# flyakon/DeepPhysiNet

Hardware: AMD Instinct MI355X
Metric: collocation-points/sec (fwd+PDE-Jacobian+bwd) (higher is better)
Workload: dtype bf16x2 (hi+lo split bf16 MFMA operands), fp32 accumulate

## Files before the change

### deepphysinet_amd/csrc/dpn_fwd_tiles.h

```cpp
#pragma once

namespace ts {
constexpr int kVecFloats = kNumVecs * 256 + 4;
template <int NS>
struct Cfg {
    static constexpr int kXBytes = 16 * 2 * NS * 1024;
    static constexpr int kVecOff = kXBytes;
    static constexpr int kRedOff = kVecOff + kVecFloats * 4;
    static constexpr int kLdsBytes = kRedOff + 4 * 64 * 4;
};

DEV void barrier_lds() {
    __builtin_amdgcn_fence(__ATOMIC_RELEASE, "workgroup", "local");
    __builtin_amdgcn_s_barrier();
    __builtin_amdgcn_fence(__ATOMIC_ACQUIRE, "workgroup", "local");
}

struct NoSide { DEV void operator()(int) const {} };

#ifdef TS_ABL_NOSINCOS
template <int NS> DEV void ts_sincos(float th, float& s, float& c) { s = th; c = th * 0.5f; }
#else
template <int NS> DEV void ts_sincos(float th, float& s, float& c) { sincos_t<NS>(th, s, c); }
#endif
// ... 181 lines not shown
#pragma unroll
    for (int q = 0; q < 4; ++q) {
        float s, co;
        ts_sincos<NS>(xi * a.freqs[8 * (ks & 3) + 4 * h + q], s, co);
        frag_set2<NS>(f, q, s, co);
    }
}
template <int NS, class Args>
DEV void pe6_frag(Frag<NS>& f, const Args& a, const int ks, const int h, const int64_t pc, const float g = 1.0f) {
    const float v = a.coord_data[pc * 6 + (ks >> 1)];
#pragma unroll
    for (int q = 0; q < 4; ++q) {
        float s, co;
        ts_sincos<NS>(v * a.freqs[32 + 8 * (ks & 1) + 4 * h + q], s, co);
        frag_set2<NS>(f, q, g * s, g * co);
    }
}
template <int NS, class Args>
DEV void pe6_frag_dot(Frag<NS>& f, const Args& a, const int ks, const int h, const int64_t pc, const float* bv, float& dot) {
    const float v = a.coord_data[pc * 6 + (ks >> 1)];
    const f32x4* b4 = reinterpret_cast<const f32x4*>(bv + 16 * ks + 8 * h);
    const f32x4 b0 = b4[0], b1 = b4[1];
    const float bb[8] = {b0[0], b0[1], b0[2], b0[3], b1[0], b1[1], b1[2], b1[3]};
#pragma unroll
    for (int q = 0; q < 4; ++q) {
        float s, co;
        ts_sincos<NS>(v * a.freqs[32 + 8 * (ks & 1) + 4 * h + q], s, co);
        frag_set2<NS>(f, q, s, co);
        dot = fmaf(s, bb[2 * q], dot);
        dot = fmaf(co, bb[2 * q + 1], dot);
    }
}
template <int NS, class Args>
DEV void z0_frag(Frag<NS>& f, const Args& a, const int ks, const int h, const int64_t pc, const float g, const float gjc) {
    const int c = ks >> 2;
    const float* src = (c == 0) ? a.x : (c == 1) ? a.y : a.t;
    const float d1 = (c == 0) ? a.geo.dx : (c == 1) ? a.geo.dy : a.geo.pred_t_span;
    const float d2 = (c == 0) ? a.geo.lon_m1 : (c == 1) ? a.geo.lat_m1 : 1.0f;
    const float xi = src[pc] / d1 / d2;
#pragma unroll
    for (int q = 0; q < 4; ++q) {
        const float fr = a.freqs[8 * (ks & 3) + 4 * h + q];
        float s, co;
        ts_sincos<NS>(xi * fr, s, co);
        const float gf = gjc * fr;
        frag_set2<NS>(f, q, fmaf(g, s, gf * co), fmaf(g, co, -gf * s));
    }
}
template <int NS, class Args>
DEV void dpe_tile(float (&d)[16], const Args& a, const int c, const int t, const int h, const int64_t pc) {
    const float* src = (c == 0) ? a.x : (c == 1) ? a.y : a.t;
    const float d1 = (c == 0) ? a.geo.dx : (c == 1) ? a.geo.dy : a.geo.pred_t_span;
    const float d2 = (c == 0) ? a.geo.lon_m1 : (c == 1) ? a.geo.lat_m1 : 1.0f;
    const float xi = src[pc] / d1 / d2;
#pragma unroll
    for (int rp = 0; rp < 8; ++rp) {
        const int r = 2 * rp;
        const float fr = a.freqs[8 * ((2 * t + (r >> 3)) & 3) + 4 * h + ((r & 7) >> 1)];
        float s, co;
        ts_sincos<NS>(xi * fr, s, co);
        d[r] = fr * co;
        d[r + 1] = -fr * s;
    }
}
template <int NS, class Args>
DEV void z0_frag_derivs(Frag<NS>& f, const Args& a, const int ks, const int h, const int64_t pc, const float g, const float gjc, const float ghc) {
    const int c = ks >> 2;
    const float* src = (c == 0) ? a.x : (c == 1) ? a.y : a.t;
    const float d1 = (c == 0) ? a.geo.dx : (c == 1) ? a.geo.dy : a.geo.pred_t_span;
    const float d2 = (c == 0) ? a.geo.lon_m1 : (c == 1) ? a.geo.lat_m1 : 1.0f;
    const float xi = src[pc] / d1 / d2;
#pragma unroll
    for (int q = 0; q < 4; ++q) {
        const float fr = a.freqs[8 * (ks & 3) + 4 * h + q];
        float s, co;
        ts_sincos<NS>(xi * fr, s, co);
        const float gf = gjc * fr;
        const float gs = fmaf(-ghc * fr, fr, g);
        frag_set2<NS>(f, q, fmaf(gs, s, gf * co), fmaf(gs, co, -gf * s));
// ... 38 lines not shown
```

### deepphysinet_amd/csrc/dpn_layout.h

```cpp
#pragma once

#if defined(__HIPCC__)
#define DPN_HD __host__ __device__ constexpr
#else
#define DPN_HD constexpr
#endif

namespace dpn {

constexpr int kNets = 6;
constexpr int kHidden = 256;
constexpr int kPe = 192;
constexpr int kW1Stride = 193;
constexpr int kW2Stride = 257;

DPN_HD int drow32(int r, int h) { return (r & 3) + 8 * (r >> 2) + 4 * h; }
DPN_HD int chain_ch(int ks, int h, int e) { return 16 * ks + 8 * (e >> 2) + 4 * h + (e & 3); }

DPN_HD int pe3_angle(int ks, int h, int e) { return 8 * ks + 4 * h + (e >> 1); }
DPN_HD int pe3_ch(int ks, int h, int e) { return (pe3_angle(ks, h, e) & 31) * 6 + (e & 1) * 3 + (pe3_angle(ks, h, e) >> 5); }
DPN_HD int pe6_ch(int ks, int h, int e) { return (pe3_angle(ks, h, e) & 15) * 12 + (e & 1) * 6 + (pe3_angle(ks, h, e) >> 4); }

DPN_HD int gpe_row_to_pe3_ch(int rho) {
    const int T = rho >> 5, i = rho & 31;
    const int r = (i & 3) + 4 * (i >> 3), h = (i >> 2) & 1;
    return pe3_ch(2 * T + (r >> 3), h, r & 7);
}

constexpr int kS0 = 0;
constexpr int kS1 = kS0 + 8 * 12;
constexpr int kS2 = kS1 + 8 * 28;
constexpr int kS3 = kS2 + 8 * 16;
constexpr int kS4 = kS3 + 8 * 16;
constexpr int kS5 = kS4 + 8 * 16;
constexpr int kPackKB = kS5 + 6 * 16;
enum { kVecB1 = 0, kVecCvec, kVecBf1, kVecU, kVecWo, kVecB2BdE_unused, kNumVecs = 6 };
DPN_HD long pack_bytes_per_net(int ns) { return (long)kPackKB * 1024 * ns + kNumVecs * 1024 + 16; }

constexpr int kF0 = kS0, kFA = kS1, kFB = kS1 + 8 * 16, kFAT = kS2, kF5 = kS5;
static_assert(kFB + 8 * 12 == kS2 && kFAT + 8 * 16 == kS3, "fused form fits the block");
enum { kVecC2 = kVecCvec, kVecA2 = kVecBf1, kVecBv = kVecB2BdE_unused };

DPN_HD bool wgrad_coop_is_y(int ns, int wave, int j) { return j < ns || (j < 2 * ns && wave < 4); }
DPN_HD int wgrad_coop_piece(int ns, int issue, int wave, int j) {
    const int xlo = issue - 2 * ns, xhi = (16 - 4 * xlo) / 4;
    if (j < ns) return 16 + 12 * j + wave;
    if (wave < 4) return j < 2 * ns ? 16 + 12 * (j - ns) + 8 + wave : xlo * wave + (j - 2 * ns);
    return j - ns < xhi ? 4 * xlo + xhi * (wave - 4) + (j - ns) : -1;
}

}
```

### deepphysinet_amd/csrc/dpn_point.hip

```cpp
#include "dpn_point_common.h"

template <int NS>
struct Frag {
    u32x4 w[NS];
};
template <int NS>
DEV void frag_set2(Frag<NS>& f, const int p, float a, float b) {
    const u32 hi = pack2(a, b);
    f.w[0][p] = hi;
    if constexpr (NS == 2) f.w[1][p] = pack2(a - bf_lo(hi), b - bf_hi(hi));
}


DEV void sincos_precise(float th, float& s, float& c) {
    const float k = rintf(th * 0.63661977236758134f);
    float r = fmaf(k, -1.5707963705062866f, th);
    r = fmaf(k, 4.371138828673793e-08f, r);
    const float r2 = r * r;
    float sp = fmaf(r2, 2.7183114939898219064e-6f, -1.9839334836096632576e-4f);
    sp = fmaf(sp, r2, 8.3333293858894631756e-3f);
    sp = fmaf(sp, r2, -1.6666666641626524100e-1f);
    sp = fmaf(sp * r2, r, r);
    float cp = fmaf(r2, 2.4433157826443582e-5f, -1.3887316255057415e-3f);
    cp = fmaf(cp, r2, 4.1666645683529456e-2f);
// ... 273 lines not shown
    }
}
DEV float lds_read_f32(unsigned addr) {
    float r;
    asm volatile("ds_read_b32 %0, %1\n\ts_waitcnt lgkmcnt(0)" : "=&v"(r) : "v"(addr) : "memory");
    return r;
}

DEV void store_d_as_k(const KMat& m, int net, int ns, int s, int64_t tile32, int ct, int lane, const f32x16& d) {
    uint4 a, b;
    a.x = pack2(d[0], d[1]); a.y = pack2(d[2], d[3]); a.z = pack2(d[4], d[5]); a.w = pack2(d[6], d[7]);
    b.x = pack2(d[8], d[9]); b.y = pack2(d[10], d[11]); b.z = pack2(d[12], d[13]); b.w = pack2(d[14], d[15]);
    typedef __attribute__((ext_vector_type(4))) unsigned int u32x4_t;
#ifdef TS_ABL_NOSTORE
    asm volatile("" ::"v"(a.x), "v"(a.y), "v"(a.z), "v"(a.w), "v"(b.x), "v"(b.y), "v"(b.z), "v"(b.w));
    return;
#endif
    __builtin_nontemporal_store(u32x4_t{a.x, a.y, a.z, a.w}, reinterpret_cast<u32x4_t*>(kmat_ptr(m, net, ns, s, tile32, ct, lane, 0)));
    __builtin_nontemporal_store(u32x4_t{b.x, b.y, b.z, b.w}, reinterpret_cast<u32x4_t*>(kmat_ptr(m, net, ns, s, tile32, ct, lane, 1)));
}
template <int NS, int NSTORE>
DEV void store_tile_k(const KMat& m, int net, int64_t tile32, int ct, const Lane& L, const Frag<NS>& f0, const Frag<NS>& f1, bool partial) {
#pragma unroll
    for (int s = 0; s < NSTORE; ++s) {
        u32x4 a0 = f0.w[s], a1 = f1.w[s];
        if (partial && !L.valid) { a0 = (u32x4)0u; a1 = (u32x4)0u; }
        f32x16 d = (f32x16)0.f;
        d = mfma(as_bf(a0), as_bf(L.idA), d);
        d = mfma(as_bf(a1), as_bf(L.idB), d);
        store_d_as_k(m, net, NSTORE, s, tile32, ct, L.lane, d);
    }
}

struct FwdArgs {
    const float *x, *y, *t, *coord_data, *freqs, *pe_in;
    int64_t n, n_pad;
    DpnGeometry geo;
    const char* packed;
    float* out_n;
    float* jac_n;
    void* saved;
    const float* ref;
#ifdef DPN_TIMELINE
    unsigned* timeline;
#endif
};

#ifdef DPN_TIMELINE
#define DPN_STAMP(I)                                                                                          \
    do {                                                                                                      \
        unsigned long long t_;                                                                                \
        asm volatile("s_memtime %0\n\ts_waitcnt lgkmcnt(0)" : "=s"(t_)::"memory");                            \
        asm volatile("v_writelane_b32 %0, %1, %2" : "+v"(tl) : "s"((u32)t_), "n"(I));                         \
    } while (0)
#else
#define DPN_STAMP(I) do { } while (0)
#endif

#ifdef DPN_FWD_PHASES
#define DPN_PH_AFTER_MMA do { u32 c4_; DPN_PH_CLOCK(c4_); pipe.ph[3] += c4_ - pipe.pc0; pipe.pc0 = c4_; } while (0)
#else
#define DPN_PH_AFTER_MMA do { } while (0)
#endif
#define DPN_STEP(C, NK, SWAP, ACT, ACC, EPI_PREV)                                    \
    do {                                                                             \
        DPN_STAMP(2 + (C));                                                          \
// ... 161 lines not shown
```

### deepphysinet_amd/csrc/dpn_point_common.h

```cpp
#pragma once
#include "dpn_device.h"

DEV void dma16(const char* gsrc_lane, char* lds_wave_base) {
    __builtin_amdgcn_global_load_lds((const __attribute__((address_space(1))) void*)(gsrc_lane),
                                     (__attribute__((address_space(3))) void*)(lds_wave_base), 16, 0, 0);
}
template <int OFF> DEV void dma16_at(const char* gsrc_lane, char* lds_wave_base) {
    __builtin_amdgcn_global_load_lds((const __attribute__((address_space(1))) void*)(gsrc_lane),
                                     (__attribute__((address_space(3))) void*)(lds_wave_base), 16, OFF, 0);
}
DEV void dma16_nt(const char* gsrc_lane, char* lds_wave_base) {
    __builtin_amdgcn_global_load_lds((const __attribute__((address_space(1))) void*)(gsrc_lane),
                                     (__attribute__((address_space(3))) void*)(lds_wave_base), 16, 0, 2);
}
DEV void dma4(const char* gsrc_lane, char* lds_wave_base) {
    __builtin_amdgcn_global_load_lds((const __attribute__((address_space(1))) void*)(gsrc_lane),
                                     (__attribute__((address_space(3))) void*)(lds_wave_base), 4, 0, 0);
}
template <int N> DEV void wait_vmcnt() { asm volatile("s_waitcnt vmcnt(%0)" ::"n"(N) : "memory"); }

struct KMat {
    char* base;
    int64_t tiles32;
    int ct_per_tile;
};
DEV char* kmat_ptr(const KMat& m, int net, int ns, int s, int64_t tile32, int ct, int lane, int kk) {
    return m.base + (((int64_t)net * ns + s) * m.tiles32 + tile32) * (m.ct_per_tile * 2048) + ((kk * m.ct_per_tile + ct) * 64 + lane) * 16;
}

struct SavedView {
    KMat T1;
    KMat M2;
    uint4* m1;
};
DEV SavedView saved_view(void* base, int64_t n_pad, int ns) {
    SavedView s;
    char* b = reinterpret_cast<char*>(base);
    const int64_t mat = (int64_t)kNets * ns * n_pad * 512;
    const int64_t tiles32 = n_pad / 32;
    s.T1 = KMat{b, tiles32, 8};
    s.M2 = KMat{b + mat, tiles32, 8};
    s.m1 = reinterpret_cast<uint4*>(b + mat + (int64_t)kNets * n_pad * 512);
    return s;
}
DPN_HD int64_t saved_state_bytes(int64_t n_pad, int ns) { return (int64_t)kNets * ns * n_pad * 512 + (int64_t)kNets * n_pad * 512 + (int64_t)kNets * n_pad * 32; }

struct OperandView {
    KMat Z1;
    KMat Z0;
    KMat PE6;
    float* gnet;
};
DEV OperandView operand_view(void* base, int64_t n_pad, int ns) {
    OperandView o;
    char* b = reinterpret_cast<char*>(base);
    const int64_t m256 = (int64_t)kNets * ns * n_pad * 512, m192 = (int64_t)kNets * ns * n_pad * 384, t192 = (int64_t)ns * n_pad * 384;
    const int64_t tiles32 = n_pad / 32;
    o.Z1 = KMat{b, tiles32, 8};
    o.Z0 = KMat{b + m256, tiles32, 6};
    o.PE6 = KMat{b + m256 + m192, tiles32, 6};
    o.gnet = reinterpret_cast<float*>(b + m256 + m192 + t192);
    return o;
}
static inline int64_t operand_bytes(int64_t n_pad, int ns) { return (int64_t)kNets * ns * n_pad * 512 + (int64_t)(kNets + 1) * ns * n_pad * 384 + (int64_t)kNets * n_pad * 4 + 1024; }

static inline int64_t pad_points(int64_t n) { return ((n + 127) / 128) * 128; }
static inline bool use_tiles(const char* knob, int prec, bool has_pe_in) {
    const char* force = getenv(knob);
    return (force ? (force[0] == 't') : (prec == 2)) && !has_pe_in;
}
```

### deepphysinet_amd/csrc/dpn_ring_kernels.inc

```

template <int NS>
#if DPN_DERIV
__global__ __launch_bounds__(256, 1) void dpn_fwd_deriv_kernel(FwdArgs a, float* hess_n, float* d3_n) {
#else
__global__ __launch_bounds__(256, 1) void dpn_fwd_kernel(FwdArgs a) {
#endif
    __shared__ __attribute__((aligned(16))) char lds_w[Pipe<NS>::kRing * Pipe<NS>::kSlotBytes];

    const int net = blockIdx.y;
    const int wave = threadIdx.x >> 6;
    const int64_t tile32 = (int64_t)blockIdx.x * 4 + wave;
    const char* pk = a.packed + (long)net * pack_bytes_per_net(NS);
    __shared__ __attribute__((aligned(16))) float lds_vec_store[kNumVecs * 256 + 4];
#ifdef DPN_TIMELINE
    u32 tl = 0;
    DPN_STAMP(0);
#endif
    {
        const float* gv = reinterpret_cast<const float*>(pk + (long)kPackKB * 1024 * NS);
        for (int i = threadIdx.x; i < kNumVecs * 256 + 4; i += 256) lds_vec_store[i] = gv[i];
    }
    const unsigned lds_vec = (unsigned)(uintptr_t)(__attribute__((address_space(3))) float*)lds_vec_store;
    Lane L;
    lane_init(L, a.x, a.y, a.t, a.n, a.freqs, a.geo, tile32);
// ... 227 lines not shown
    __shared__ __attribute__((aligned(16))) float lds_vec_store[kNumVecs * 256 + 4];
    {
        const float* gv = reinterpret_cast<const float*>(pk + (long)kPackKB * 1024 * NS);
        for (int i = threadIdx.x; i < kNumVecs * 256 + 4; i += 256) lds_vec_store[i] = gv[i];
    }
    const unsigned lds_vec = (unsigned)(uintptr_t)(__attribute__((address_space(3))) float*)lds_vec_store;
    Lane L;
    lane_init(L, a.x, a.y, a.t, a.n, a.freqs, a.geo, tile32);
    const int h = L.h;
    const int64_t pc = L.valid ? L.pt : (a.n - 1);
    float cd6[6];
#pragma unroll
    for (int c = 0; c < 6; ++c) cd6[c] = a.coord_data[pc * 6 + c];
    const float gsc = a.g_scale ? a.g_scale[0] : 1.0f;
    const float g = L.valid ? gsc * a.g_out[pc * 6 + net] : 0.f;
    float gj[3] = {0.f, 0.f, 0.f};
    if (a.g_jxi && L.valid) {
#pragma unroll
        for (int c = 0; c < 3; ++c) gj[c] = gsc * a.g_jxi[(pc * 6 + net) * 3 + c];
    }
#if DPN_DERIV
    float gh[3] = {0.f, 0.f, 0.f};
    if (g_hxi && L.valid) {
#pragma unroll
        for (int c = 0; c < 3; ++c) gh[c] = gsc * g_hxi[(pc * 6 + net) * 3 + c];
    }
#endif
    SavedView sv = saved_view(a.saved, a.n_pad, NS);
    OperandView ov = operand_view(a.operands, a.n_pad, NS);
    const int64_t tiles32 = a.n_pad / 32;
    const uint4 m1v = sv.m1[((int64_t)net * tiles32 + tile32) * 64 + L.lane];
    const u32 m1w[4] = {m1v.x, m1v.y, m1v.z, m1v.w};
    if (h == 0) ov.gnet[(int64_t)net * a.n_pad + tile32 * 32 + L.j] = g;

    Pipe<NS> pipe;
    __syncthreads();
    pipe.init(pk, lds_w, 8);
    pipe.prime();

    f32x16 acc[8];
    Frag<NS> actA[16];
#ifdef DPN_TIMELINE
    u32 tl = 0;
#endif
    auto epi1 = [&](const int T) __attribute__((always_inline)) {
#pragma unroll
        for (int r = 0; r < 16; r += 2) {
            const u32 bits = m1w[T >> 1] >> (16 * (T & 1) + r);
            frag_set2<NS>(actA[2 * T + (r >> 3)], (r & 7) >> 1, (bits & 1u) ? acc[T][r] : 0.f, (bits & 2u) ? acc[T][r + 1] : 0.f);
        }
        store_tile_k<NS, NS>(ov.Z1, net, tile32, T, L, actA[2 * T], actA[2 * T + 1], false);
    };
    {
        Frag<NS> z0[12];
        if (net == 0) {
            build_pe6<NS>(L, cd6, z0, 1.0f);
#pragma unroll
            for (int ct = 0; ct < 6; ++ct) store_tile_k<NS, NS>(ov.PE6, 0, tile32, ct, L, z0[2 * ct], z0[2 * ct + 1], false);
        }
        if (a.pe_in) load_pe3<NS>(a.pe_in + pc * kPe, h, z0, g);
#if DPN_DERIV
        else build_z0_derivs<NS>(L, z0, g, gj, gh);
#else
        else build_pe3<NS, true>(L, z0, g, gj);
#endif
#pragma unroll
        for (int ct = 0; ct < 6; ++ct) store_tile_k<NS, NS>(ov.Z0, net, tile32, ct, L, z0[2 * ct], z0[2 * ct + 1], false);
#pragma unroll
        for (int T = 0; T < 8; ++T) {
            acc_init_vec(acc[T], lds_vec, kVecB1, h, T, g);
            if (T == 0) DPN_STEP(T, 12, false, z0, acc[T], (void)0);
            else DPN_STEP(T, 12, false, z0, acc[T], epi1(T - 1));
        }
        epi1(7);
        pipe.drain();
    }
}
```

### deepphysinet_amd/csrc/dpn_tiles_kernels.inc

```

template <int NS>
#if DPN_DERIV
__global__ __launch_bounds__(256, 2) void dpn_fwd_tiles_deriv_kernel(FwdArgs a, float* hess_n, float* d3_n) {
#else
__global__ __launch_bounds__(256, 2) void dpn_fwd_tiles_kernel(FwdArgs a) {
#endif
    using C = ts::Cfg<NS>;
    __shared__ __attribute__((aligned(16))) char lds[C::kLdsBytes];
    const int net = blockIdx.y;
    const int w = __builtin_amdgcn_readfirstlane(threadIdx.x >> 6);
    const int lane = threadIdx.x & 63, j = lane & 31, h = lane >> 5;
    const char* pk = a.packed + (long)net * pack_bytes_per_net(NS);
#if TS_PRIO == 2
    __builtin_amdgcn_s_setprio(1);
#endif
    TS_STAMP(0);
    float* vec = reinterpret_cast<float*>(lds + C::kVecOff);
    float* red = reinterpret_cast<float*>(lds + C::kRedOff);
    char* xl = lds + lane * 16;
    {
        const u32x4* gv = reinterpret_cast<const u32x4*>(pk + (long)kPackKB * 1024 * NS);
        static_assert(ts::kVecFloats % 4 == 0 && ts::kVecFloats / 4 <= 512, "vector block");
        const int i0 = threadIdx.x, i1 = threadIdx.x + 256;
        const u32x4 v0 = gv[i0];
// ... 289 lines not shown
    const int lane = threadIdx.x & 63, j = lane & 31, h = lane >> 5;
    TS_STAMP(0);
    const char* pk = a.packed + (long)net * pack_bytes_per_net(NS);
#if TS_PRIO == 2
    __builtin_amdgcn_s_setprio(1);
#endif
    float* vec = reinterpret_cast<float*>(lds + kXBytes) - kVecB1 * 256;
    char* xl = lds + lane * 16;
    {
        const float* gv = reinterpret_cast<const float*>(pk + (long)kPackKB * 1024 * NS) + kVecB1 * 256;
        reinterpret_cast<float*>(lds + kXBytes)[threadIdx.x] = gv[threadIdx.x];
    }
    auto chunk = [&](const int kb) __attribute__((always_inline)) { return pk + (long)kb * 1024 * NS; };
    ts::Head<NS, 2> H;
    ts::gemm_head<NS, 12, 2>(chunk(kS0 + 2 * w * 12), lane, H);
    const int64_t tile0 = (int64_t)blockIdx.x * 2;
    const int64_t tiles32 = a.n_pad / 32;
    int64_t pc[2];
    float g[2];
    const float gsc = a.g_scale ? a.g_scale[0] : 1.0f;
#pragma unroll
    for (int p = 0; p < 2; ++p) {
        const int64_t pt = (tile0 + p) * 32 + j;
        const bool valid = pt < a.n;
        pc[p] = valid ? pt : (a.n - 1);
        g[p] = valid ? gsc * a.g_out[pc[p] * 6 + net] : 0.f;
    }
    const ts::Ident I = ts::make_ident(j, h);
    SavedView sv = saved_view(a.saved, a.n_pad, NS);
    OperandView ov = operand_view(a.operands, a.n_pad, NS);
    u32 m1w[2];
#pragma unroll
    for (int p = 0; p < 2; ++p) m1w[p] = reinterpret_cast<const u32*>(sv.m1 + ((int64_t)net * tiles32 + tile0 + p) * 64 + lane)[w];
    if (w == 0) {
        const int64_t pt = (tile0 + h) * 32 + j;
        ov.gnet[(int64_t)net * a.n_pad + pt] = (pt < a.n) ? gsc * a.g_out[pt * 6 + net] : 0.f;
    }
#pragma unroll
    for (int uu = 0; uu < 3; ++uu) {
        const int u = 3 * w + uu, ct = u >> 1, p = u & 1;
        const float gp = p ? g[1] : g[0];
        const int64_t pcp = p ? pc[1] : pc[0];
        float gjc = 0.f;
        if (a.g_jxi && ((tile0 + p) * 32 + j) < a.n) gjc = gsc * a.g_jxi[(pcp * 6 + net) * 3 + (ct >> 1)];
        Frag<NS> f0, f1;
#if DPN_DERIV
        float ghc = 0.f;
        if (g_hxi && ((tile0 + p) * 32 + j) < a.n) ghc = gsc * g_hxi[(pcp * 6 + net) * 3 + (ct >> 1)];
        ts::z0_frag_derivs<NS>(f0, a, 2 * ct, h, pcp, gp, gjc, ghc);
        ts::z0_frag_derivs<NS>(f1, a, 2 * ct + 1, h, pcp, gp, gjc, ghc);
#else
        ts::z0_frag<NS>(f0, a, 2 * ct, h, pcp, gp, gjc);
        ts::z0_frag<NS>(f1, a, 2 * ct + 1, h, pcp, gp, gjc);
#endif
        ts::x_store<NS>(xl, 2 * ct, p, f0);
        ts::x_store<NS>(xl, 2 * ct + 1, p, f1);
        ts::save_tile_k<NS, NS>(ov.Z0, net, tile0 + p, ct, lane, I, false, f0, f1);
    }
    TS_STAMP(1);
    ts::barrier_lds();
    TS_STAMP(2);
    f32x16 acc[2][2];
#pragma unroll
    for (int t = 0; t < 2; ++t)
#pragma unroll
        for (int p = 0; p < 2; ++p) ts::acc_init(acc[t][p], vec, kVecB1, h, 2 * w + t, g[p]);
    ts::gemm<NS, 12, 2, false, ts::NoSide, false>(chunk(kS0 + 2 * w * 12), xl, lane, H, acc);
    TS_STAMP(3);
#pragma unroll
    for (int t = 0; t < 2; ++t)
#pragma unroll
        for (int p = 0; p < 2; ++p) {
            Frag<NS> F0, F1;
#pragma unroll
            for (int r = 0; r < 16; r += 2) {
                const u32 bits = m1w[p] >> (16 * t + r);
                frag_set2<NS>(r < 8 ? F0 : F1, (r & 7) >> 1, (bits & 1u) ? acc[t][p][r] : 0.f, (bits & 2u) ? acc[t][p][r + 1] : 0.f);
            }
            ts::save_tile_k<NS, NS>(ov.Z1, net, tile0 + p, 2 * w + t, lane, I, false, F0, F1);
        }
    TS_STAMP(4);
    if (net != 0) return;
#pragma unroll
    for (int uu = 0; uu < 3; ++uu) {
        const int u = 3 * w + uu, ct = u >> 1, p = u & 1;
        const int64_t pcp = p ? pc[1] : pc[0];
        Frag<NS> f0, f1;
        ts::pe6_frag<NS>(f0, a, 2 * ct, h, pcp);
        ts::pe6_frag<NS>(f1, a, 2 * ct + 1, h, pcp);
// ... 5 lines not shown
```

### deepphysinet_amd/csrc/dpn_wgrad.hip

```cpp
#include <type_traits>

#include "dpn_point_common.h"

DEV u16 f2bf(float x) {
    unsigned u = __float_as_uint(x);
    u += 0x7FFFu + ((u >> 16) & 1u);
    return (u16)(u >> 16);
}
DEV float bf2f(u16 b) { return __uint_as_float(((unsigned)b) << 16); }

struct PackArgs {
    DpnNetPtrs net[kNets];
    char* packed;
    int ns;
    int form;
    int n_fields;
    long heads_stride, evec_stride, packed_stride;
};
DEV DpnNetPtrs pack_net(const PackArgs& a, const int net, const int field) {
    DpnNetPtrs P = a.net[net];
    P.w1b1 += field * a.heads_stride;
    P.w2b2 += field * a.heads_stride;
    P.evec += field * a.evec_stride;
    return P;
// ... 224 lines not shown
#ifdef DPN_WGRAD_PHASES
    unsigned* phases;
#endif
};
#ifdef DPN_WGRAD_PHASES
#define DPN_WG_CLOCK(V) do { unsigned long long t_; asm volatile("s_memtime %0\n\ts_waitcnt lgkmcnt(0)" : "=s"(t_)::"memory"); V = (u32)t_; } while (0)
#else
#define DPN_WG_CLOCK(V) do { } while (0)
#endif

template <int NS, int PROD>
struct WgradShape {
    static constexpr int nct = PROD < 2 ? 8 : 6;
    static constexpr int nsx = PROD == 3 ? NS : 1;
    static constexpr int kX = nsx * 16384, kYPlane = nct * 2048, kY = NS * kYPlane;
    static constexpr int kPieces = (kX + kY) / 1024;
    static constexpr int kIssue = (kPieces + 7) / 8;
    static constexpr int kPad = kIssue * 8 - kPieces;
    static constexpr int kGOff = kX + kY;
    static constexpr int kPadOff = kGOff + 8 * 256;
    static constexpr int kSlot = kPadOff + (kPad ? 1024 : 0);
    static constexpr int PER_TILE = kIssue + 1;
    static constexpr int RING = (160 * 1024) / kSlot < 5 ? (160 * 1024) / kSlot : 5;
};
template <int NS>
constexpr int wgrad_lds_bytes() {
    int m = 0;
    const int v[3] = {WgradShape<NS, 1>::RING * WgradShape<NS, 1>::kSlot, WgradShape<NS, 2>::RING * WgradShape<NS, 2>::kSlot,
                      WgradShape<NS, 3>::RING * WgradShape<NS, 3>::kSlot};
    for (int k = 0; k < 3; ++k) m = v[k] > m ? v[k] : m;
    return m;
}

template <int NS, int PROD>
DEV void wgrad_body(const WgradArgs& a, char* lds, const int split, const int net) {
    using S = WgradShape<NS, PROD>;
    constexpr int nct = S::nct, nsx = S::nsx, kSlot = S::kSlot, RING = S::RING, PER_TILE = S::PER_TILE, ncol = nct * 32;
    const int64_t tiles = a.n_pad / 32;
    const int64_t per = (tiles + a.splits[PROD] - 1) / a.splits[PROD];
    const int64_t t0 = (int64_t)split * per;
    int64_t t1 = t0 + per < tiles ? t0 + per : tiles;
    if (t1 < t0) t1 = t0;

    const int lane = threadIdx.x & 63, wave = __builtin_amdgcn_readfirstlane(threadIdx.x >> 6);
#ifdef DPN_WGRAD_2X4_ONLY
    constexpr bool kWide = true;
#else
    constexpr bool kWide = nct == 8;
#endif
    constexpr int MT = kWide ? 4 : 2, NT = kWide ? 2 : 3;
    const int wm = kWide ? wave >> 2 : wave >> 1, wn = kWide ? wave & 3 : wave & 1;
    const int i = lane & 31, h = lane >> 5;
    const bool active = wn * NT < nct;
    SavedView sv = saved_view(a.saved, a.n_pad, NS);
    OperandView ov = operand_view(a.operands, a.n_pad, NS);
    const char* xb = (PROD == 3) ? sv.T1.base : sv.M2.base;
    static_assert(PROD >= 1 && PROD <= 3, "products: 1 = M2^T Z1, 2 = M2^T G6, 3 = T1^T Z0");
    const char* yb = (PROD == 1) ? ov.Z1.base : (PROD == 2) ? ov.PE6.base : ov.Z0.base;
    const int64_t ynet = (PROD == 2) ? 0 : net;
    const float* gnet = ov.gnet + (int64_t)net * a.n_pad;

    constexpr bool kCoop = PROD == 2;
    static_assert(!kCoop || (2 * nct == 12 && nsx == 1 && S::kIssue >= 2 * NS), "product 2: 12 column pairs over 8 waves");
    const bool two_pairs = wave < 4;
    const char* pbase[S::kIssue];
    int pstride[S::kIssue], pdst[S::kIssue];
#pragma unroll
    for (int j = 0; j < S::kIssue; ++j) {
        int q = wave + 8 * j;
        if constexpr (kCoop) q = wgrad_coop_piece(NS, S::kIssue, wave, j);
        if (S::kPad && (kCoop ? q < 0 : q >= S::kPieces)) {
            pbase[j] = xb + ((int64_t)net * nsx * tiles + (t0 < tiles ? t0 : 0)) * 16384; pstride[j] = 0; pdst[j] = S::kPadOff;
        } else if (q < nsx * 16) {
            pbase[j] = xb + ((int64_t)net * nsx + q / 16) * tiles * 16384 + (q % 16) * 1024; pstride[j] = 16384; pdst[j] = q * 1024;
        } else {
            const int qy = q - nsx * 16;
            pbase[j] = yb + (ynet * NS + qy / (2 * nct)) * tiles * S::kYPlane + (qy % (2 * nct)) * 1024; pstride[j] = S::kYPlane; pdst[j] = q * 1024;
        }
    }
    auto issue = [&](int64_t tile, int slot) __attribute__((always_inline)) {
        char* sl = lds + slot * kSlot;
#pragma unroll
        for (int j = 0; j < S::kIssue; ++j) {
            if (kCoop && wgrad_coop_is_y(NS, wave, j)) dma16(pbase[j] + tile * pstride[j] + lane * 16, sl + pdst[j]);
            else dma16_nt(pbase[j] + tile * pstride[j] + lane * 16, sl + pdst[j]);
        }
        dma4(reinterpret_cast<const char*>(gnet + tile * 32) + lane * 4, sl + S::kGOff + wave * 256);
    };

    f32x16 acc[MT][NT];
#pragma unroll
    for (int m = 0; m < MT; ++m)
#pragma unroll
        for (int n2 = 0; n2 < NT; ++n2) acc[m][n2] = (f32x16)0.f;
    float vecA[MT], vecB[NT], gsum = 0.f;
#pragma unroll
    for (int m = 0; m < MT; ++m) vecA[m] = 0.f;
#pragma unroll
    for (int n2 = 0; n2 < NT; ++n2) vecB[n2] = 0.f;
    auto owns_row = [&](const int m) __attribute__((always_inline)) { return (kWide && nct == 6) ? wn == m % 3 : wn == m; };
    auto owns_col = [&](const int n2) __attribute__((always_inline)) { return wm == n2; };

    const unsigned lds_base = (unsigned)(uintptr_t)(__attribute__((address_space(3))) char*)lds;
    auto rd128 = [&](u32x4& v, const unsigned addr) __attribute__((always_inline)) {
        asm volatile("ds_read_b128 %0, %1" : "=v"(v) : "v"(addr) : "memory");
    };
    auto compute = [&](const int slot_) __attribute__((always_inline)) {
        const unsigned buf = lds_base + slot_ * kSlot;
        const unsigned gl = buf + S::kGOff + wave * 256;
        constexpr int KB = (NS == 1) ? 2 : 1;
        u32x4 gqa[KB][2], faa[KB][nsx][MT], fba[KB][NS][NT];
        const unsigned baseG = gl + h * 16;
        const unsigned baseA = buf + wm * (MT * 1024) + lane * 16, baseB = buf + S::kX + wn * (NT * 1024) + lane * 16;
        auto rd128o = [&](u32x4& v, const unsigned base, const int off) __attribute__((always_inline)) {
            asm volatile("ds_read_b128 %0, %1 offset:%2" : "=v"(v) : "v"(base), "i"(off) : "memory");
        };
        auto issue_reads = [&](const int kk, const int b) __attribute__((always_inline)) {
            if constexpr (!kCoop) {
                rd128o(gqa[b][0], baseG, 64 * kk);
                rd128o(gqa[b][1], baseG, 64 * kk + 32);
            }
#pragma unroll
            for (int s2 = 0; s2 < nsx; ++s2)
#pragma unroll
                for (int m = 0; m < MT; ++m) rd128o(faa[b][s2][m], baseA, s2 * 16384 + (kk * 8 + m) * 1024);
#pragma unroll
            for (int s2 = 0; s2 < NS; ++s2)
#pragma unroll
                for (int n2 = 0; n2 < NT; ++n2) rd128o(fba[b][s2][n2], baseB, s2 * S::kYPlane + (kk * nct + n2) * 1024);
        };
        constexpr int kReads = (kCoop ? 0 : 2) + MT * nsx + NT * NS;
        if constexpr (NS == 1) { issue_reads(0, 0); issue_reads(1, 1); }
#pragma unroll
        for (int kk = 0; kk < 2; ++kk) {
            const int b = (NS == 1) ? kk : 0;
            if constexpr (NS == 2) issue_reads(kk, 0);
            u32x4 (&fa)[nsx][MT] = faa[b];
            u32x4 (&fb)[NS][NT] = fba[b];
            u32x4& gq0 = gqa[b][0];
            u32x4& gq1 = gqa[b][1];
            if (NS == 1 && kk == 0) asm volatile("s_waitcnt lgkmcnt(%0)" :: "n"(kReads) : "memory");
            else asm volatile("s_waitcnt lgkmcnt(0)" ::: "memory");
            if constexpr (kCoop) gq0 = gq1 = (u32x4)0u;
            else asm volatile("" : "+v"(gq0), "+v"(gq1));
            asm volatile("" : "+v"(fa[0][0]), "+v"(fa[0][1]), "+v"(fb[0][0]), "+v"(fb[0][1]));
            if constexpr (MT == 4) asm volatile("" : "+v"(fa[0][2]), "+v"(fa[0][3]));
            if constexpr (NT == 3) asm volatile("" : "+v"(fb[0][2]));
            if constexpr (NS == 2) asm volatile("" : "+v"(fb[1][0]), "+v"(fb[1][1]));
            if constexpr (NS == 2 && NT == 3) asm volatile("" : "+v"(fb[1][2]));
            if constexpr (nsx == 2) asm volatile("" : "+v"(fa[1][0]), "+v"(fa[1][1]));
            if constexpr (nsx == 2 && MT == 4) asm volatile("" : "+v"(fa[1][2]), "+v"(fa[1][3]));
            const float gp[8] = {__uint_as_float(gq0[0]), __uint_as_float(gq0[1]), __uint_as_float(gq0[2]), __uint_as_float(gq0[3]),
                                 __uint_as_float(gq1[0]), __uint_as_float(gq1[1]), __uint_as_float(gq1[2]), __uint_as_float(gq1[3])};
            if (PROD == 1 && wave == 0 && i == 0) {
#pragma unroll
                for (int e = 0; e < 8; ++e) gsum += gp[e];
            }
#pragma unroll
            for (int m = 0; m < MT; ++m) {
                if (owns_row(m) && PROD != 2) {
                    float d = 0.f;
#pragma unroll
                    for (int s2 = 0; s2 < nsx; ++s2) {
#pragma unroll
                        for (int p = 0; p < 4; ++p) { d = fmaf(bf_lo(fa[s2][m][p]), gp[2 * p], d); d = fmaf(bf_hi(fa[s2][m][p]), gp[2 * p + 1], d); }
                    }
                    vecA[m] += d;
                }
#pragma unroll
                for (int n2 = 0; n2 < NT; ++n2) {
                    if constexpr (NS == 2) {
                        acc[m][n2] = mfma(as_bf(fa[0][m]), as_bf(fb[1][n2]), acc[m][n2]);
                        if constexpr (nsx == 2) acc[m][n2] = mfma(as_bf(fa[1][m]), as_bf(fb[0][n2]), acc[m][n2]);
                    }
                    acc[m][n2] = mfma(as_bf(fa[0][m]), as_bf(fb[0][n2]), acc[m][n2]);
                }
// ... 16 lines not shown
    auto form = [&](const int slot_) __attribute__((always_inline)) {
        const unsigned buf = lds_base + slot_ * kSlot;
        const unsigned baseG = buf + S::kGOff + wave * 256 + h * 16, baseY = buf + S::kX + wave * 1024 + lane * 16;
        auto pair = [&](auto q_) __attribute__((always_inline)) {
            constexpr int q = decltype(q_)::value;
            const unsigned ay = baseY + q * 8192, ag = baseG + ((wave + 8 * q) >= nct ? 64 : 0);
            u32x4 t[2], gq0, gq1;
            rd128(gq0, ag);
            asm volatile("ds_read_b128 %0, %1 offset:32" : "=v"(gq1) : "v"(ag) : "memory");
            rd128(t[0], ay);
            if constexpr (NS == 2) asm volatile("ds_read_b128 %0, %1 offset:%2" : "=v"(t[1]) : "v"(ay), "i"(S::kYPlane) : "memory");
            asm volatile("s_waitcnt lgkmcnt(0)" ::: "memory");
            asm volatile("" : "+v"(gq0), "+v"(gq1), "+v"(t[0]));
            if constexpr (NS == 2) asm volatile("" : "+v"(t[1]));
            const float gp[8] = {__uint_as_float(gq0[0]), __uint_as_float(gq0[1]), __uint_as_float(gq0[2]), __uint_as_float(gq0[3]),
                                 __uint_as_float(gq1[0]), __uint_as_float(gq1[1]), __uint_as_float(gq1[2]), __uint_as_float(gq1[3])};
#pragma unroll
            for (int p = 0; p < 4; ++p) {
                float v0 = bf_lo(t[0][p]), v1 = bf_hi(t[0][p]);
                if constexpr (NS == 2) { v0 += bf_lo(t[1][p]); v1 += bf_hi(t[1][p]); }
                const float z0 = gp[2 * p] * v0, z1 = gp[2 * p + 1] * v1;
                const u32 hi = pack2(z0, z1);
                t[0][p] = hi;
                if constexpr (NS == 2) t[1][p] = pack2(z0 - bf_lo(hi), z1 - bf_hi(hi));
            }
            asm volatile("ds_write_b128 %0, %1" :: "v"(ay), "v"(t[0]) : "memory");
            if constexpr (NS == 2) asm volatile("ds_write_b128 %0, %1 offset:%2" :: "v"(ay), "v"(t[1]), "i"(S::kYPlane) : "memory");
        };
        pair(std::integral_constant<int, 0>{});
        if (two_pairs) pair(std::integral_constant<int, 1>{});
        asm volatile("s_waitcnt lgkmcnt(0)" ::: "memory");
    };

    const int64_t tl = t1 > t0 ? t1 - 1 : t0;
#pragma unroll
    for (int r = 0; r < RING - 1; ++r) issue(t0 + r < t1 ? t0 + r : tl, r);
    int slot = 0;
#ifdef DPN_WGRAD_PHASES
    u32 c0 = 0, c1 = 0, c2 = 0, c3 = 0, c4 = 0, ph_wait = 0, ph_bar = 0, ph_issue = 0, ph_comp = 0;
#endif
    for (int64_t tile = t0; tile < t1; ++tile) {
        DPN_WG_CLOCK(c0);
        wait_vmcnt<(RING - 2) * PER_TILE>();
        if constexpr (kCoop) form(slot);
        DPN_WG_CLOCK(c1);
        __builtin_amdgcn_s_barrier();
        DPN_WG_CLOCK(c2);
        {
            const int64_t nt = tile + RING - 1;
            issue(nt < t1 ? nt : tl, (slot + RING - 1) % RING);
        }
        DPN_WG_CLOCK(c3);
        if (active) compute(slot);
        DPN_WG_CLOCK(c4);
#ifdef DPN_WGRAD_PHASES
        ph_wait += c1 - c0; ph_bar += c2 - c1; ph_issue += c3 - c2; ph_comp += c4 - c3;
#endif
        slot = (slot + 1) % RING;
    }
#ifdef DPN_WGRAD_PHASES
    if (a.phases && lane == 0) {
        unsigned* o = a.phases + (((int64_t)blockIdx.y * gridDim.x + blockIdx.x) * 8 + wave) * 8;
        o[0] = ph_wait; o[1] = ph_bar; o[2] = ph_issue; o[3] = ph_comp; o[4] = (unsigned)(t1 - t0); o[5] = PROD;
    }
#endif
    wait_vmcnt<0>();
    __builtin_amdgcn_s_barrier();
    float* part = a.partials + ((int64_t)split * kNets + net) * kPartFloats;
    float* out = part + part_off(PROD);
    if (active) {
#pragma unroll
        for (int m = 0; m < MT; ++m)
#pragma unroll
            for (int n2 = 0; n2 < NT; ++n2)
#pragma unroll
                for (int r = 0; r < 16; ++r) {
                    const int rr = wm * (MT * 32) + 32 * m + drow32(r, h);
// ... 2 lines not shown
                }
    }
#pragma unroll
    for (int m = 0; m < MT; ++m) {
        const float v = vecA[m] + __shfl_xor(vecA[m], 32);
        if (owns_row(m) && h == 0) {
            const int rr = wm * (MT * 32) + 32 * m + i;
            if (PROD == 1) part[kPartVec + 2 * 256 + rr] = v;
            if (PROD == 3) part[kPartVec + 3 * 256 + rr] = v;
        }
    }
    if (PROD == 1 && wave == 0) {
        const float gs = gsum + __shfl_xor(gsum, 32);
        if (lane == 0) part[kPartVec + 4 * 256] = gs;
    }
    if (PROD != 3 && active) {
        const int qo = kPartVec + (PROD == 1 ? 5 : 6) * 256;
#pragma unroll
        for (int n2 = 0; n2 < NT; ++n2) {
            const float v = vecB[n2] + __shfl_xor(vecB[n2], 32);
            if (owns_col(n2) && h == 0) part[qo + wn * (NT * 32) + 32 * n2 + i] = v;
        }
    }
}

template <int NS>
__global__ __launch_bounds__(512, 2) void dpn_wgrad_kernel(WgradArgs a) {
    __shared__ __attribute__((aligned(16))) char lds[wgrad_lds_bytes<NS>()];
    int prod = 1, split = blockIdx.x;
    const int net = blockIdx.y;
    while (prod < 3 && split >= a.splits[prod]) { split -= a.splits[prod]; ++prod; }
    if (prod == 1) wgrad_body<NS, 1>(a, lds, split, net);
    else if (prod == 2) wgrad_body<NS, 2>(a, lds, split, net);
    else wgrad_body<NS, 3>(a, lds, split, net);
}

struct FinishArgs {
    DpnNetPtrs net[kNets];
    DpnNetGradPtrs grad[kNets];
    const char* packed;
    const float* partials;
    float* scratch_s1;
    float* scratch_s2;
    float* scratch_mv;
    float* scratch_u;
    float* scratch_q1;
    float* scratch_q6;
    float* scratch_sg;
    float* scratch_rp;
    int splits[4], ns;
    int64_t n;
};

DEV int slot_of_ch(int ch) { return (ch & ~15) + 8 * ((ch >> 2) & 1) + 4 * ((ch >> 3) & 1) + (ch & 3); }
DEV int slot_of_pe3(int orig) {
    const int f = orig / 6, fn = (orig % 6) / 3, c = orig % 3;
    const int a = 32 * c + f;
    const int ks = a >> 3, h = (a >> 2) & 1, p = a & 3;
    return 16 * ks + 8 * h + 2 * p + fn;
}
DEV int slot_of_pe6(int orig) {
    const int f = orig / 12, fn = (orig % 12) / 6, c6 = orig % 6;
    const int a = 16 * c6 + f;
    const int ks = a >> 3, h = (a >> 2) & 1, p = a & 3;
    return 16 * ks + 8 * h + 2 * p + fn;
}

// ... 377 lines not shown
```

Baseline: 33.12 million.

## Store Z0 as a shared sin/cos table and rebuild per-net operands inside wgrad

In hi+lo mode the forward kernels stop storing a per-net Z0 operand for every net. They store one shared sin/cos table (three-way bf16 split, one column tile written per net) plus per-net g_j coefficients, and a header records the form used and the frequencies. The wgrad product-3 kernel reads this header and uses a new TAB variant. That variant loads the shared table and g/gj, then rebuilds g*sin + gj*f*cos in LDS (form_z0) before the MFMA. The aim is to cut the HBM write and read traffic for Z0 across the six nets, at the cost of extra ALU and LDS work in wgrad and a more complex piece schedule.

```diff
diff --git a/deepphysinet_amd/csrc/dpn_fwd_tiles.h b/deepphysinet_amd/csrc/dpn_fwd_tiles.h
--- a/deepphysinet_amd/csrc/dpn_fwd_tiles.h
+++ b/deepphysinet_amd/csrc/dpn_fwd_tiles.h
@@ -237,7 +237,7 @@
     }
 }
 template <int NS, class Args>
-DEV void z0_frag(Frag<NS>& f, const Args& a, const int ks, const int h, const int64_t pc, const float g, const float gjc) {
+DEV void z0_frag(Frag<NS>& f, const Args& a, const int ks, const int h, const int64_t pc, const float g, const float gjc, float (&sc)[8]) {
     const int c = ks >> 2;
     const float* src = (c == 0) ? a.x : (c == 1) ? a.y : a.t;
     const float d1 = (c == 0) ? a.geo.dx : (c == 1) ? a.geo.dy : a.geo.pred_t_span;
@@ -250,6 +250,7 @@
         ts_sincos<NS>(xi * fr, s, co);
         const float gf = gjc * fr;
         frag_set2<NS>(f, q, fmaf(g, s, gf * co), fmaf(g, co, -gf * s));
+        sc[2 * q] = s; sc[2 * q + 1] = co;
     }
 }
 template <int NS, class Args>
diff --git a/deepphysinet_amd/csrc/dpn_layout.h b/deepphysinet_amd/csrc/dpn_layout.h
--- a/deepphysinet_amd/csrc/dpn_layout.h
+++ b/deepphysinet_amd/csrc/dpn_layout.h
@@ -49,4 +49,15 @@
     return j - ns < xhi ? 4 * xlo + xhi * (wave - 4) + (j - ns) : -1;
 }
 
+
+DPN_HD int wgrad_z0_ct(int wave) { return wave < 4 ? wave : 4 + (wave & 1); }
+DPN_HD int wgrad_z0_pairs(int wave) { return wave < 4 ? 2 : 1; }
+DPN_HD int wgrad_z0_kk(int wave, int q) { return wave < 4 ? q : (wave - 4) >> 1; }
+DPN_HD bool wgrad_z0_is_y(int wave, int j) { return j < 2 * wgrad_z0_pairs(wave); }
+DPN_HD int wgrad_z0_piece(int wave, int j) {
+    if (wgrad_z0_is_y(wave, j)) return 32 + 12 * (j & 1) + 6 * wgrad_z0_kk(wave, j >> 1) + wgrad_z0_ct(wave);
+    return wave < 4 ? 3 * wave + (j - 4) : 12 + 5 * (wave - 4) + (j - 2);
 }
+DPN_HD int z0_freq_index(int ct, int jj) { return 16 * (ct & 1) + (jj >> 1); }
+
+}
diff --git a/deepphysinet_amd/csrc/dpn_point.hip b/deepphysinet_amd/csrc/dpn_point.hip
--- a/deepphysinet_amd/csrc/dpn_point.hip
+++ b/deepphysinet_amd/csrc/dpn_point.hip
@@ -329,6 +329,35 @@
     }
 }
 
+DEV void store_table_k(const KMat& z0, const int64_t tile32, const int ct, const int lane, const u32x4& idA, const u32x4& idB, const float (&v0)[8],
+                       const float (&v1)[8]) {
+    u32x4 a0[3], a1[3];
+#pragma unroll
+    for (int p = 0; p < 4; ++p) {
+        auto split = [&](const float x, const float y, u32x4 (&a)[3]) __attribute__((always_inline)) {
+            const u32 w0 = pack2(x, y);
+            const float rx = x - bf_lo(w0), ry = y - bf_hi(w0);
+            const u32 w1 = pack2(rx, ry);
+            a[0][p] = w0; a[1][p] = w1; a[2][p] = pack2(rx - bf_lo(w1), ry - bf_hi(w1));
+        };
+        split(v0[2 * p], v0[2 * p + 1], a0);
+        split(v1[2 * p], v1[2 * p + 1], a1);
+    }
+    f32x16 d = (f32x16)0.f;
+#pragma unroll
+    for (int q = 0; q < 3; ++q) {
+        d = mfma(as_bf(a0[q]), as_bf(idA), d);
+        d = mfma(as_bf(a1[q]), as_bf(idB), d);
+    }
+    typedef __attribute__((ext_vector_type(4))) float f32x4_t;
+#pragma unroll
+    for (int kk = 0; kk < 2; ++kk)
+#pragma unroll
+        for (int s = 0; s < 2; ++s)
+            __builtin_nontemporal_store(f32x4_t{d[8 * kk + 4 * s], d[8 * kk + 4 * s + 1], d[8 * kk + 4 * s + 2], d[8 * kk + 4 * s + 3]},
+                                        reinterpret_cast<f32x4_t*>(kmat_ptr(z0, 0, 2, s, tile32, ct, lane, kk)));
+}
+
 struct FwdArgs {
     const float *x, *y, *t, *coord_data, *freqs, *pe_in;
     int64_t n, n_pad;
diff --git a/deepphysinet_amd/csrc/dpn_point_common.h b/deepphysinet_amd/csrc/dpn_point_common.h
--- a/deepphysinet_amd/csrc/dpn_point_common.h
+++ b/deepphysinet_amd/csrc/dpn_point_common.h
@@ -50,7 +50,10 @@
     KMat Z0;
     KMat PE6;
     float* gnet;
+    float* gj;
+    unsigned* hdr;
 };
+constexpr unsigned kZ0Stored = 0u, kZ0Table = 1u;
 DEV OperandView operand_view(void* base, int64_t n_pad, int ns) {
     OperandView o;
     char* b = reinterpret_cast<char*>(base);
@@ -60,7 +63,14 @@
     o.Z0 = KMat{b + m256, tiles32, 6};
     o.PE6 = KMat{b + m256 + m192, tiles32, 6};
     o.gnet = reinterpret_cast<float*>(b + m256 + m192 + t192);
+    o.gj = reinterpret_cast<float*>(b + m256 + t192);
+    o.hdr = reinterpret_cast<unsigned*>(b + m256 + m192 + t192 + (int64_t)kNets * n_pad * 4 + 256);
     return o;
+}
+DEV void write_operand_header(const OperandView& o, const unsigned form, const float* freqs) {
+    if (blockIdx.x != 0 || blockIdx.y != 0 || threadIdx.x >= 32) return;
+    if (threadIdx.x == 0) o.hdr[0] = form;
+    o.hdr[4 + threadIdx.x] = __float_as_uint(freqs[threadIdx.x]);
 }
 static inline int64_t operand_bytes(int64_t n_pad, int ns) { return (int64_t)kNets * ns * n_pad * 512 + (int64_t)(kNets + 1) * ns * n_pad * 384 + (int64_t)kNets * n_pad * 4 + 1024; }
 
diff --git a/deepphysinet_amd/csrc/dpn_ring_kernels.inc b/deepphysinet_amd/csrc/dpn_ring_kernels.inc
--- a/deepphysinet_amd/csrc/dpn_ring_kernels.inc
+++ b/deepphysinet_amd/csrc/dpn_ring_kernels.inc
@@ -283,6 +283,12 @@
     const uint4 m1v = sv.m1[((int64_t)net * tiles32 + tile32) * 64 + L.lane];
     const u32 m1w[4] = {m1v.x, m1v.y, m1v.z, m1v.w};
     if (h == 0) ov.gnet[(int64_t)net * a.n_pad + tile32 * 32 + L.j] = g;
+    const bool z0_table = NS == 2 && !DPN_DERIV && !a.pe_in;
+    write_operand_header(ov, z0_table ? kZ0Table : kZ0Stored, a.freqs);
+    if (z0_table && h == 0) {
+#pragma unroll
+        for (int c = 0; c < 3; ++c) ov.gj[((int64_t)net * 3 + c) * a.n_pad + tile32 * 32 + L.j] = gj[c];
+    }
 
     Pipe<NS> pipe;
     __syncthreads();
@@ -315,8 +321,21 @@
 #else
         else build_pe3<NS, true>(L, z0, g, gj);
 #endif
-#pragma unroll
-        for (int ct = 0; ct < 6; ++ct) store_tile_k<NS, NS>(ov.Z0, net, tile32, ct, L, z0[2 * ct], z0[2 * ct + 1], false);
+        if (z0_table) {
+#pragma unroll
+            for (int ct = 0; ct < 6; ++ct) {
+                if (ct != net) continue;
+                float v[2][8];
+#pragma unroll
+                for (int k2 = 0; k2 < 2; ++k2)
+#pragma unroll
+                    for (int p = 0; p < 4; ++p) sincos_t<NS>(L.xi[ct >> 1] * L.fr32[4 * ((2 * ct + k2) & 3) + p], v[k2][2 * p], v[k2][2 * p + 1]);
+                if constexpr (NS == 2) store_table_k(ov.Z0, tile32, ct, L.lane, L.idA, L.idB, v[0], v[1]);
+            }
+        } else {
+#pragma unroll
+            for (int ct = 0; ct < 6; ++ct) store_tile_k<NS, NS>(ov.Z0, net, tile32, ct, L, z0[2 * ct], z0[2 * ct + 1], false);
+        }
 #pragma unroll
         for (int T = 0; T < 8; ++T) {
             acc_init_vec(acc[T], lds_vec, kVecB1, h, T, g);
diff --git a/deepphysinet_amd/csrc/dpn_tiles_kernels.inc b/deepphysinet_amd/csrc/dpn_tiles_kernels.inc
--- a/deepphysinet_amd/csrc/dpn_tiles_kernels.inc
+++ b/deepphysinet_amd/csrc/dpn_tiles_kernels.inc
@@ -345,9 +345,14 @@
     u32 m1w[2];
 #pragma unroll
     for (int p = 0; p < 2; ++p) m1w[p] = reinterpret_cast<const u32*>(sv.m1 + ((int64_t)net * tiles32 + tile0 + p) * 64 + lane)[w];
+    constexpr bool kTab = NS == 2 && !DPN_DERIV;
+    write_operand_header(ov, kTab ? kZ0Table : kZ0Stored, a.freqs);
     if (w == 0) {
         const int64_t pt = (tile0 + h) * 32 + j;
         ov.gnet[(int64_t)net * a.n_pad + pt] = (pt < a.n) ? gsc * a.g_out[pt * 6 + net] : 0.f;
+    } else if (kTab) {
+        const int64_t pt = (tile0 + h) * 32 + j;
+        ov.gj[((int64_t)net * 3 + (w - 1)) * a.n_pad + pt] = (a.g_jxi && pt < a.n) ? gsc * a.g_jxi[(pt * 6 + net) * 3 + (w - 1)] : 0.f;
     }
 #pragma unroll
     for (int uu = 0; uu < 3; ++uu) {
@@ -363,11 +368,17 @@
         ts::z0_frag_derivs<NS>(f0, a, 2 * ct, h, pcp, gp, gjc, ghc);
         ts::z0_frag_derivs<NS>(f1, a, 2 * ct + 1, h, pcp, gp, gjc, ghc);
 #else
-        ts::z0_frag<NS>(f0, a, 2 * ct, h, pcp, gp, gjc);
-        ts::z0_frag<NS>(f1, a, 2 * ct + 1, h, pcp, gp, gjc);
+        float sc0[8], sc1[8];
+        ts::z0_frag<NS>(f0, a, 2 * ct, h, pcp, gp, gjc, sc0);
+        ts::z0_frag<NS>(f1, a, 2 * ct + 1, h, pcp, gp, gjc, sc1);
 #endif
         ts::x_store<NS>(xl, 2 * ct, p, f0);
         ts::x_store<NS>(xl, 2 * ct + 1, p, f1);
+#if !DPN_DERIV
+        if constexpr (NS == 2) {
+            if (ct == net) store_table_k(ov.Z0, tile0 + p, ct, lane, I.a, I.b, sc0, sc1);
+        } else
+#endif
         ts::save_tile_k<NS, NS>(ov.Z0, net, tile0 + p, ct, lane, I, false, f0, f1);
     }
     TS_STAMP(1);
diff --git a/deepphysinet_amd/csrc/dpn_wgrad.hip b/deepphysinet_amd/csrc/dpn_wgrad.hip
--- a/deepphysinet_amd/csrc/dpn_wgrad.hip
+++ b/deepphysinet_amd/csrc/dpn_wgrad.hip
@@ -280,8 +280,9 @@
     return m;
 }
 
-template <int NS, int PROD>
+template <int NS, int PROD, bool TAB = false>
 DEV void wgrad_body(const WgradArgs& a, char* lds, const int split, const int net) {
+    static_assert(!TAB || (NS == 2 && PROD == 3), "the table form of Z0: hi+lo mode, product 3");
     using S = WgradShape<NS, PROD>;
     constexpr int nct = S::nct, nsx = S::nsx, kSlot = S::kSlot, RING = S::RING, PER_TILE = S::PER_TILE, ncol = nct * 32;
     const int64_t tiles = a.n_pad / 32;
@@ -305,18 +306,28 @@
     const char* xb = (PROD == 3) ? sv.T1.base : sv.M2.base;
     static_assert(PROD >= 1 && PROD <= 3, "products: 1 = M2^T Z1, 2 = M2^T G6, 3 = T1^T Z0");
     const char* yb = (PROD == 1) ? ov.Z1.base : (PROD == 2) ? ov.PE6.base : ov.Z0.base;
-    const int64_t ynet = (PROD == 2) ? 0 : net;
+    const int64_t ynet = (PROD == 2 || TAB) ? 0 : net;
     const float* gnet = ov.gnet + (int64_t)net * a.n_pad;
-
-    constexpr bool kCoop = PROD == 2;
-    static_assert(!kCoop || (2 * nct == 12 && nsx == 1 && S::kIssue >= 2 * NS), "product 2: 12 column pairs over 8 waves");
+    const char* gsrc = reinterpret_cast<const char*>(gnet) + lane * 4;
+    float fr = 0.f;
+    if constexpr (TAB) {
+        const int ct = wgrad_z0_ct(wave);
+        if (lane >= 32) gsrc = reinterpret_cast<const char*>(ov.gj + ((int64_t)net * 3 + (ct >> 1)) * a.n_pad) + (lane - 32) * 4;
+        fr = __uint_as_float(ov.hdr[4 + z0_freq_index(ct, lane & 31)]);
+        asm volatile("" : "+v"(fr));
+    }
+
+    constexpr bool kCoop = PROD == 2 || TAB;
+    static_assert(PROD != 2 || (2 * nct == 12 && nsx == 1 && S::kIssue >= 2 * NS), "product 2: 12 column pairs over 8 waves");
+    static_assert(!TAB || (S::kIssue == 7 && S::kPad == 0 && nsx == 2), "product 3, table form: 56 pieces, seven per wave");
     const bool two_pairs = wave < 4;
     const char* pbase[S::kIssue];
     int pstride[S::kIssue], pdst[S::kIssue];
 #pragma unroll
     for (int j = 0; j < S::kIssue; ++j) {
         int q = wave + 8 * j;
-        if constexpr (kCoop) q = wgrad_coop_piece(NS, S::kIssue, wave, j);
+        if constexpr (TAB) q = wgrad_z0_piece(wave, j);
+        else if constexpr (kCoop) q = wgrad_coop_piece(NS, S::kIssue, wave, j);
         if (S::kPad && (kCoop ? q < 0 : q >= S::kPieces)) {
             pbase[j] = xb + ((int64_t)net * nsx * tiles + (t0 < tiles ? t0 : 0)) * 16384; pstride[j] = 0; pdst[j] = S::kPadOff;
         } else if (q < nsx * 16) {
@@ -330,10 +341,10 @@
         char* sl = lds + slot * kSlot;
 #pragma unroll
         for (int j = 0; j < S::kIssue; ++j) {
-            if (kCoop && wgrad_coop_is_y(NS, wave, j)) dma16(pbase[j] + tile * pstride[j] + lane * 16, sl + pdst[j]);
+            if (kCoop && (TAB ? wgrad_z0_is_y(wave, j) : wgrad_coop_is_y(NS, wave, j))) dma16(pbase[j] + tile * pstride[j] + lane * 16, sl + pdst[j]);
             else dma16_nt(pbase[j] + tile * pstride[j] + lane * 16, sl + pdst[j]);
         }
-        dma4(reinterpret_cast<const char*>(gnet + tile * 32) + lane * 4, sl + S::kGOff + wave * 256);
+        dma4(gsrc + tile * 128, sl + S::kGOff + wave * 256);
     };
 
     f32x16 acc[MT][NT];
@@ -364,7 +375,7 @@
             asm volatile("ds_read_b128 %0, %1 offset:%2" : "=v"(v) : "v"(base), "i"(off) : "memory");
         };
         auto issue_reads = [&](const int kk, const int b) __attribute__((always_inline)) {
-            if constexpr (!kCoop) {
+            if constexpr (PROD != 2) {
                 rd128o(gqa[b][0], baseG, 64 * kk);
                 rd128o(gqa[b][1], baseG, 64 * kk + 32);
             }
@@ -377,7 +388,7 @@
 #pragma unroll
                 for (int n2 = 0; n2 < NT; ++n2) rd128o(fba[b][s2][n2], baseB, s2 * S::kYPlane + (kk * nct + n2) * 1024);
         };
-        constexpr int kReads = (kCoop ? 0 : 2) + MT * nsx + NT * NS;
+        constexpr int kReads = (PROD == 2 ? 0 : 2) + MT * nsx + NT * NS;
         if constexpr (NS == 1) { issue_reads(0, 0); issue_reads(1, 1); }
 #pragma unroll
         for (int kk = 0; kk < 2; ++kk) {
@@ -389,7 +400,7 @@
             u32x4& gq1 = gqa[b][1];
             if (NS == 1 && kk == 0) asm volatile("s_waitcnt lgkmcnt(%0)" :: "n"(kReads) : "memory");
             else asm volatile("s_waitcnt lgkmcnt(0)" ::: "memory");
-            if constexpr (kCoop) gq0 = gq1 = (u32x4)0u;
+            if constexpr (PROD == 2) gq0 = gq1 = (u32x4)0u;
             else asm volatile("" : "+v"(gq0), "+v"(gq1));
             asm volatile("" : "+v"(fa[0][0]), "+v"(fa[0][1]), "+v"(fb[0][0]), "+v"(fb[0][1]));
             if constexpr (MT == 4) asm volatile("" : "+v"(fa[0][2]), "+v"(fa[0][3]));
@@ -472,6 +483,45 @@
         asm volatile("s_waitcnt lgkmcnt(0)" ::: "memory");
     };
 
+    auto form_z0 = [&](const int slot_) __attribute__((always_inline)) {
+        const unsigned buf = lds_base + slot_ * kSlot;
+        const int ct = wgrad_z0_ct(wave);
+        const unsigned baseG = buf + S::kGOff + wave * 256 + h * 16, baseY = buf + S::kX + ct * 1024;
+        const u32 sgn = (lane & 1) ? 0x80000000u : 0u;
+        auto pair = [&](const int kk) __attribute__((always_inline)) {
+            const unsigned ay = baseY + kk * (nct * 1024) + lane * 16, ap = baseY + kk * (nct * 1024) + (lane ^ 1) * 16, ag = baseG + kk * 64;
+            u32x4 gq[2], jq[2], own[2], par[2];
+            rd128(gq[0], ag);
+            asm volatile("ds_read_b128 %0, %1 offset:32" : "=v"(gq[1]) : "v"(ag) : "memory");
+            asm volatile("ds_read_b128 %0, %1 offset:128" : "=v"(jq[0]) : "v"(ag) : "memory");
+            asm volatile("ds_read_b128 %0, %1 offset:160" : "=v"(jq[1]) : "v"(ag) : "memory");
+            rd128(own[0], ay);
+            asm volatile("ds_read_b128 %0, %1 offset:%2" : "=v"(own[1]) : "v"(ay), "i"(S::kYPlane) : "memory");
+            rd128(par[0], ap);
+            asm volatile("ds_read_b128 %0, %1 offset:%2" : "=v"(par[1]) : "v"(ap), "i"(S::kYPlane) : "memory");
+            asm volatile("s_waitcnt lgkmcnt(0)" ::: "memory");
+            asm volatile("" : "+v"(gq[0]), "+v"(gq[1]), "+v"(jq[0]), "+v"(jq[1]), "+v"(own[0]), "+v"(own[1]), "+v"(par[0]), "+v"(par[1]));
+            float z[8];
+#pragma unroll
+            for (int e = 0; e < 8; ++e) {
+                const float gf = __uint_as_float(jq[e >> 2][e & 3]) * fr;
+                const float t = __uint_as_float(__float_as_uint(gf * __uint_as_float(par[e >> 2][e & 3])) ^ sgn);
+                z[e] = fmaf(__uint_as_float(gq[e >> 2][e & 3]), __uint_as_float(own[e >> 2][e & 3]), t);
+            }
+            u32x4 hi, lo;
+#pragma unroll
+            for (int p = 0; p < 4; ++p) {
+                hi[p] = pack2(z[2 * p], z[2 * p + 1]);
+                lo[p] = pack2(z[2 * p] - bf_lo(hi[p]), z[2 * p + 1] - bf_hi(hi[p]));
+            }
+            asm volatile("ds_write_b128 %0, %1" :: "v"(ay), "v"(hi) : "memory");
+            asm volatile("ds_write_b128 %0, %1 offset:%2" :: "v"(ay), "v"(lo), "i"(S::kYPlane) : "memory");
+        };
+        pair(wgrad_z0_kk(wave, 0));
+        if (two_pairs) pair(wgrad_z0_kk(wave, 1));
+        asm volatile("s_waitcnt lgkmcnt(0)" ::: "memory");
+    };
+
     const int64_t tl = t1 > t0 ? t1 - 1 : t0;
 #pragma unroll
     for (int r = 0; r < RING - 1; ++r) issue(t0 + r < t1 ? t0 + r : tl, r);
@@ -482,7 +532,8 @@
     for (int64_t tile = t0; tile < t1; ++tile) {
         DPN_WG_CLOCK(c0);
         wait_vmcnt<(RING - 2) * PER_TILE>();
-        if constexpr (kCoop) form(slot);
+        if constexpr (TAB) form_z0(slot);
+        else if constexpr (kCoop) form(slot);
         DPN_WG_CLOCK(c1);
         __builtin_amdgcn_s_barrier();
         DPN_WG_CLOCK(c2);
@@ -551,7 +602,13 @@
     while (prod < 3 && split >= a.splits[prod]) { split -= a.splits[prod]; ++prod; }
     if (prod == 1) wgrad_body<NS, 1>(a, lds, split, net);
     else if (prod == 2) wgrad_body<NS, 2>(a, lds, split, net);
-    else wgrad_body<NS, 3>(a, lds, split, net);
+    else {
+        if constexpr (NS == 2) {
+            const unsigned form = __builtin_amdgcn_readfirstlane(operand_view(a.operands, a.n_pad, NS).hdr[0]);
+            if (form == kZ0Table) { wgrad_body<NS, 3, true>(a, lds, split, net); return; }
+        }
+        wgrad_body<NS, 3>(a, lds, split, net);
+    }
 }
 
 struct FinishArgs {
```

Result: faster. 35.00 million (median of 6 runs) (+5.7%).
